# KELVIN-ASU/Lightweight-Multi-Modal-Scene-Understanding-via-Knowledge-Distillation

Hardware: AMD Instinct MI355X
Metric: PandaSet 2-class KD training frames/sec (higher is better)
Workload: dtype f32; 1 GPU; KD step: concat-fusion teacher fwd (eval) -> weighted-fusion student fwd/bwd (train BN), CE + T^2*KL(T=4) + feature-MSE, fused AdamW; random-init weights; teacher_fusion=concat, student_fusion=weighted, image=3x256x256, points_per_frame=80000, bev_grid=64x64, num_classes=2, per_gpu_batch=256, global_batch=256, parallelism=dp1

## Files before the change

### lightweight-multi-modal-scene-understanding-via-knowledge-distillation_amd/csrc/kd_lidar.hip

```cpp
#include "kd_common.h"

namespace {

struct BevGeom { float x0, xd, y0, yd; int H, W; };

__device__ __forceinline__ bool bev_cell(const float4 pt, const BevGeom g, int& cell) {
  const float xn = __fdiv_rn(__fsub_rn(pt.x, g.x0), g.xd);
  const float yn = __fdiv_rn(__fsub_rn(pt.y, g.y0), g.yd);
  const bool valid = (xn >= 0.f) && (xn <= 1.f) && (yn >= 0.f) && (yn <= 1.f);
  if (!valid) { cell = -1; return false; }
  long long ix = (long long)__fmul_rn(xn, (float)(g.W - 1));
  long long iy = (long long)__fmul_rn(yn, (float)(g.H - 1));
  ix = ix < 0 ? 0 : (ix > g.W - 1 ? g.W - 1 : ix);
  iy = iy < 0 ? 0 : (iy > g.H - 1 ? g.H - 1 : iy);
  cell = (int)(iy * g.W + ix);
  return true;
}

struct L0Args {
  const float* pts; const float* w; const float* b; float* y; float* partial;
  int64_t P; int C; int groups, slots; const int* p_dev;
};
__global__ __launch_bounds__(256) void lidar_l0_fwd_kernel(L0Args a) {
  __shared__ float red[2 * 256 * 4];
// ... 364 lines not shown
  const int64_t p = (int64_t)blockIdx.x * blockDim.x + threadIdx.x;
  if (p >= P) return;
  int c;
  if (bev_cell(kd_ld4(pts + p * 4), g, c)) {
    const int row = (int)(p / N) * (g.H * g.W) + c;
    row_of_point[p] = row;
    rank[p] = atomicAdd(counts + row, 1);
  } else {
    row_of_point[p] = -1;
  }
}

__global__ __launch_bounds__(256) void scan_block_sums_kernel(const int* __restrict__ v, int* __restrict__ bsum, int64_t n) {
  __shared__ int red[256];
  const int64_t base = (int64_t)blockIdx.x * SCAN_CHUNK;
  int s = 0;
  for (int i = threadIdx.x; i < SCAN_CHUNK; i += 256)
    if (base + i < n) s += v[base + i];
  red[threadIdx.x] = s;
  __syncthreads();
  for (int off = 128; off > 0; off >>= 1) {
    if ((int)threadIdx.x < off) red[threadIdx.x] += red[threadIdx.x + off];
    __syncthreads();
  }
  if (threadIdx.x == 0) bsum[blockIdx.x] = red[0];
}

__global__ __launch_bounds__(1024) void scan_bsums_kernel(int* bsum, int nb) {
  __shared__ int sh[1024];
  int carry = 0;
  for (int base = 0; base < nb; base += 1024) {
    const int i = base + (int)threadIdx.x;
    const int v = i < nb ? bsum[i] : 0;
    sh[threadIdx.x] = v;
    __syncthreads();
    for (int off = 1; off < 1024; off <<= 1) {
      const int t = (int)threadIdx.x >= off ? sh[threadIdx.x - off] : 0;
      __syncthreads();
      sh[threadIdx.x] += t;
      __syncthreads();
    }
    if (i < nb) bsum[i] = carry + sh[threadIdx.x] - v;
    carry += sh[1023];
    __syncthreads();
  }
}

__global__ __launch_bounds__(256) void scan_apply_kernel(int* v, const int* __restrict__ bsum, int64_t n) {
  __shared__ int sh[256];
  const int64_t base = (int64_t)blockIdx.x * SCAN_CHUNK + (int64_t)threadIdx.x * 8;
  int x[8];
  int tot = 0;
#pragma unroll
  for (int j = 0; j < 8; ++j) { x[j] = base + j < n ? v[base + j] : 0; tot += x[j]; }
  sh[threadIdx.x] = tot;
  __syncthreads();
  for (int off = 1; off < 256; off <<= 1) {
    const int t = (int)threadIdx.x >= off ? sh[threadIdx.x - off] : 0;
    __syncthreads();
    sh[threadIdx.x] += t;
    __syncthreads();
  }
  int run = bsum[blockIdx.x] + sh[threadIdx.x] - tot;
#pragma unroll
  for (int j = 0; j < 8; ++j) {
    if (base + j < n) v[base + j] = run;
    run += x[j];
  }
}

__global__ void seg_fill_kernel(const int* __restrict__ row_of_point, const int* __restrict__ rank,
                                const int* __restrict__ start, int* __restrict__ perm, int64_t P) {
  const int64_t p = (int64_t)blockIdx.x * blockDim.x + threadIdx.x;
  if (p >= P) return;
  const int row = row_of_point[p];
  if (row >= 0) perm[start[row] + rank[p]] = (int)p;
}

constexpr int SORT_BLK = 1024;
constexpr int SORT_MAX_BINS = 36865;

__global__ __launch_bounds__(SORT_BLK) void stable_count_kernel(const float* __restrict__ pts, int* __restrict__ key_out,
                                                                int* __restrict__ lrank_out, int* __restrict__ T, int64_t N,
                                                                int nblk, BevGeom g) {
  extern __shared__ int hist[];
  const int HW = g.H * g.W, nb = HW + 1;
  const int tid = threadIdx.x, lane = tid & 63, wave = tid >> 6;
  const int b = blockIdx.x / nblk, blk = blockIdx.x % nblk;
  for (int i = tid; i < nb; i += SORT_BLK) hist[i] = 0;
  const int64_t n = (int64_t)blk * SORT_BLK + tid;
  const bool act = n < N;
  const int64_t p = (int64_t)b * N + (act ? n : 0);
  int key = -1;
  if (act) {
    int c;
    key = bev_cell(kd_ld4(pts + p * 4), g, c) ? c : HW;
  }
  int r = 0, cnt = 0;
#pragma unroll 16
  for (int j = 0; j < 64; ++j) {
    const int kj = __shfl(key, j);
    cnt += kj == key ? 1 : 0;
    r += (kj == key && j < lane) ? 1 : 0;
  }
  __syncthreads();
  int lr = 0;
  for (int w = 0; w < SORT_BLK / 64; ++w) {
    if (wave == w && act) lr = hist[key] + r;
    __syncthreads();
    if (wave == w && act && r == cnt - 1) hist[key] += cnt;
    __syncthreads();
  }
  if (act) { key_out[p] = key; lrank_out[p] = lr; }
  int* Tb = T + ((int64_t)b * nblk + blk) * nb;
  for (int i = tid; i < nb; i += SORT_BLK) Tb[i] = hist[i];
}

__global__ void stable_prefix_kernel(int* T, int* __restrict__ counts, int* __restrict__ inv, int B, int nblk, int HW) {
  const int nb = HW + 1;
  const int64_t idx = (int64_t)blockIdx.x * blockDim.x + threadIdx.x;
  if (idx == 0) counts[(int64_t)B * HW] = 0;
  if (idx >= (int64_t)B * nb) return;
  const int b = (int)(idx / nb), key = (int)(idx % nb);
  int run = 0;
  for (int blk = 0; blk < nblk; ++blk) {
    int* t = T + ((int64_t)b * nblk + blk) * nb + key;
    const int v = *t;
    *t = run;
    run += v;
  }
  if (key < HW) counts[(int64_t)b * HW + key] = run; else inv[b] = run;
}

__global__ void stable_inv_base_kernel(const int* __restrict__ seg_start, int* inv, int B, int64_t ncells) {
  if (threadIdx.x != 0 || blockIdx.x != 0) return;
  int run = seg_start[ncells];
  for (int b = 0; b < B; ++b) { const int v = inv[b]; inv[b] = run; run += v; }
}

__global__ void stable_fill_kernel(const float* __restrict__ pts, const int* __restrict__ key, const int* __restrict__ lrank,
                                   const int* __restrict__ T, const int* __restrict__ seg_start, const int* __restrict__ inv_base,
                                   float* __restrict__ pts_sorted, int* __restrict__ row_sorted, int* __restrict__ perm,
                                   int64_t P, int64_t N, int nblk, int HW) {
  const int64_t p = (int64_t)blockIdx.x * blockDim.x + threadIdx.x;
  if (p >= P) return;
  const int b = (int)(p / N), blk = (int)((p % N) / SORT_BLK), k = key[p];
  const int base = k < HW ? seg_start[(int64_t)b * HW + k] : inv_base[b];
  const int64_t pos = (int64_t)base + T[((int64_t)b * nblk + blk) * (HW + 1) + k] + lrank[p];
  kd_st4(pts_sorted + pos * 4, kd_ld4(pts + p * 4));
  row_sorted[pos] = k < HW ? b * HW + k : -1;
  if (perm) perm[pos] = (int)p;
}

constexpr int WIDE_MAX_DIM = 4096;

__device__ __forceinline__ void wave_same_key(int key, int lane, int& below, int& all) {
  below = 0; all = 0;
#pragma unroll 16
  for (int j = 0; j < 64; ++j) {
    const int kj = __shfl(key, j);
    all += kj == key ? 1 : 0;
    below += (kj == key && j < lane) ? 1 : 0;
  }
}

__device__ __forceinline__ int block_stable_rank(int key, bool act, int below, int all, int* hist) {
  const int wave = threadIdx.x >> 6;
  int lr = 0;
  for (int w = 0; w < SORT_BLK / 64; ++w) {
    if (wave == w && act) lr = hist[key] + below;
    __syncthreads();
    if (wave == w && act && below == all - 1) hist[key] += all;
    __syncthreads();
  }
  return lr;
}

template <int PASS>
__global__ __launch_bounds__(SORT_BLK) void wide_count_kernel(const float* __restrict__ pts, int* __restrict__ cell_io,
                                                              int* __restrict__ lrank_out, int* __restrict__ T,
                                                              int* counts, int64_t N, int nblk, BevGeom g) {
  extern __shared__ int hist[];
  const int nd = PASS == 0 ? g.W : g.H + 1;
  const int tid = threadIdx.x, lane = tid & 63;
  const int b = blockIdx.x / nblk, blk = blockIdx.x % nblk;
  for (int i = tid; i < nd; i += SORT_BLK) hist[i] = 0;
  const int64_t n = (int64_t)blk * SORT_BLK + tid;
  const bool act = n < N;
  const int64_t p = (int64_t)b * N + (act ? n : 0);
  int cell = -1;
  if (act) {
    if (PASS == 0) bev_cell(kd_ld4(pts + p * 4), g, cell); else cell = cell_io[p];
  }
  const int key = !act ? -1 : PASS == 0 ? (cell >= 0 ? cell % g.W : 0) : (cell >= 0 ? cell / g.W : g.H);
  int below, all;
  wave_same_key(key, lane, below, all);
  if (PASS == 0) {
    int cbelow, call;
    wave_same_key(cell, lane, cbelow, call);
    if (cell >= 0 && cbelow == 0) atomicAdd(counts + (int64_t)b * g.H * g.W + cell, call);
  }
  __syncthreads();
  const int lr = block_stable_rank(key, act, below, all, hist);
  if (act) {
    if (PASS == 0) cell_io[p] = cell;
    lrank_out[p] = lr;
  }
  int* Tb = T + ((int64_t)b * nblk + blk) * nd;
  for (int i = tid; i < nd; i += SORT_BLK) Tb[i] = hist[i];
}

__global__ void wide_prefix_kernel(int* T, int* __restrict__ tot, int* __restrict__ last_tot, int B, int nblk, int nd) {
  const int64_t idx = (int64_t)blockIdx.x * blockDim.x + threadIdx.x;
  if (idx >= (int64_t)B * nd) return;
  const int b = (int)(idx / nd), d = (int)(idx % nd);
  int run = 0;
  for (int blk = 0; blk < nblk; ++blk) {
    int* t = T + ((int64_t)b * nblk + blk) * nd + d;
    const int v = *t;
    *t = run;
    run += v;
  }
  tot[idx] = run;
  if (last_tot && d == nd - 1) last_tot[b] = run;
}

__global__ __launch_bounds__(64) void wide_frame_scan_kernel(int* tot, int nd) {
  int* t = tot + (int64_t)blockIdx.x * nd;
  const int lane = threadIdx.x;
  int carry = 0;
  for (int base = 0; base < nd; base += 64) {
    const int i = base + lane;
    const int v = i < nd ? t[i] : 0;
    int incl = v;
#pragma unroll
    for (int off = 1; off < 64; off <<= 1) {
      const int u = __shfl_up(incl, off);
      if (lane >= off) incl += u;
    }
    if (i < nd) t[i] = carry + incl - v;
    carry += __shfl(incl, 63);
  }
}

__global__ void wide_mid_kernel(const int* __restrict__ cell, const int* __restrict__ lrank, const int* __restrict__ T,
                                const int* __restrict__ off, int* __restrict__ mid_id, int* __restrict__ mid_cell, int64_t P,
                                int64_t N, int nblk, int W) {
  const int64_t p = (int64_t)blockIdx.x * blockDim.x + threadIdx.x;
  if (p >= P) return;
  const int b = (int)(p / N), blk = (int)((p % N) / SORT_BLK), c = cell[p];
  const int d = c >= 0 ? c % W : 0;
  const int64_t pos = (int64_t)b * N + off[(int64_t)b * W + d] + T[((int64_t)b * nblk + blk) * W + d] + lrank[p];
  mid_id[pos] = (int)p;
  mid_cell[pos] = c;
}

__global__ void wide_fill_kernel(const float* __restrict__ pts, const int* __restrict__ mid_id, const int* __restrict__ mid_cell,
                                 const int* __restrict__ lrank, const int* __restrict__ T, const int* __restrict__ off,
                                 const int* __restrict__ seg_start, const int* __restrict__ inv_base,
                                 float* __restrict__ pts_sorted, int* __restrict__ row_sorted, int* __restrict__ perm,
                                 int64_t P, int64_t N, int nblk, int H, int W) {
  const int64_t q = (int64_t)blockIdx.x * blockDim.x + threadIdx.x;
  if (q >= P) return;
  const int b = (int)(q / N), blk = (int)((q % N) / SORT_BLK), c = mid_cell[q], p = mid_id[q];
  const int nd = H + 1, d = c >= 0 ? c / W : H;
  const int64_t HW = (int64_t)H * W;
  const int in_digit = T[((int64_t)b * nblk + blk) * nd + d] + lrank[q];
  const int64_t pos = c >= 0 ? (int64_t)seg_start[b * HW] + off[(int64_t)b * nd + d] + in_digit : (int64_t)inv_base[b] + in_digit;
  kd_st4(pts_sorted + pos * 4, kd_ld4(pts + (int64_t)p * 4));
  row_sorted[pos] = c >= 0 ? (int)(b * HW + c) : -1;
  if (perm) perm[pos] = p;
}

struct SegArgs {
  const float* y; const float* sc; const float* sh; int act;
  const int* start; const int* perm;
  float* grid; const float* dout; const float* mean; const float* invstd;
  float* G; float* partial; int64_t ncells; int C;
  int long_len; const int* rowid; float* cnt; int prow0;
  float* rawmax; uint8_t* holders;
};
constexpr int SEG_LONG = 256;
constexpr int SEG_HOLD_SWEEP = 255;

template <int VEC> struct SegVec;
template <> struct SegVec<1> { typedef float type; };
template <> struct SegVec<2> { typedef float2 type; };
template <> struct SegVec<4> { typedef float4 type; };

template <int VEC> __device__ __forceinline__ void seg_ld(float (&r)[VEC], const float* p) {
  const typename SegVec<VEC>::type v = *reinterpret_cast<const typename SegVec<VEC>::type*>(p);
  __builtin_memcpy(r, &v, sizeof(v));
}
template <int VEC> __device__ __forceinline__ void seg_st(float* p, const float (&r)[VEC]) {
  typename SegVec<VEC>::type v;
  __builtin_memcpy(&v, r, sizeof(v));
  *reinterpret_cast<typename SegVec<VEC>::type*>(p) = v;
}

template <int VEC, bool PERM>
__global__ __launch_bounds__(256) void seg_max_fwd_kernel(SegArgs a) {
  const int lane = threadIdx.x & 63;
  const int c0 = lane * VEC;
  float sc[VEC], sh[VEC];
  seg_ld<VEC>(sc, a.sc + c0);
  seg_ld<VEC>(sh, a.sh + c0);
// ... 287 lines not shown
  seg_stat_rows_out<VEC>(a, red, blockIdx.x, wave, c0, s1, s2);
}

template <int VEC, int MODE>
__global__ __launch_bounds__(256) void seg_long_kernel(SegArgs a) {
  __shared__ float red[4][2][64 * VEC];
  const int lane = threadIdx.x & 63, wave = threadIdx.x >> 6;
  const int c0 = lane * VEC;
  float sc[VEC], sh[VEC], mu[VEC], inv[VEC], s1[VEC], s2[VEC];
  seg_ld<VEC>(sc, a.sc + c0);
  seg_ld<VEC>(sh, a.sh + c0);
#pragma unroll
  for (int j = 0; j < VEC; ++j) { s1[j] = 0.f; s2[j] = 0.f; mu[j] = 0.f; inv[j] = 0.f; }
  if (MODE == 2) { seg_ld<VEC>(mu, a.mean + c0); seg_ld<VEC>(inv, a.invstd + c0); }
  const int nvalid = __builtin_amdgcn_readfirstlane(a.start[a.ncells]);
  const int64_t nw = (int64_t)gridDim.x * 4;
  for (int64_t w = (int64_t)blockIdx.x * 4 + wave; w * 64 < nvalid; w += nw) {
    const int i0 = (int)(w * 64), i1 = i0 + 64 < nvalid ? i0 + 64 : nvalid;
    const int cf = __builtin_amdgcn_readfirstlane(a.rowid[i0]), cl = __builtin_amdgcn_readfirstlane(a.rowid[i1 - 1]);
    const bool lf = a.start[cf + 1] - a.start[cf] > a.long_len, ll = a.start[cl + 1] - a.start[cl] > a.long_len;
    if (!lf && !ll) continue;
    int i = i0;
    while (i < i1) {
      const int cell = __builtin_amdgcn_readfirstlane(a.rowid[i]);
      const int cs = __builtin_amdgcn_readfirstlane(a.start[cell]), ce = __builtin_amdgcn_readfirstlane(a.start[cell + 1]);
      const int rend = ce < i1 ? ce : i1;
      if (ce - cs <= a.long_len) { i = rend; continue; }
      float acc[VEC], mx[VEC], share[VEC];
#pragma unroll
      for (int j = 0; j < VEC; ++j) { acc[j] = 0.f; mx[j] = 0.f; share[j] = 0.f; }
      if (MODE >= 1) seg_ld<VEC>(mx, a.grid + (int64_t)cell * a.C + c0);
      if (MODE == 2) {
        float d[VEC], n[VEC];
        seg_ld<VEC>(d, a.dout + (int64_t)cell * a.C + c0);
        seg_ld<VEC>(n, a.cnt + (int64_t)cell * a.C + c0);
#pragma unroll
        for (int j = 0; j < VEC; ++j) share[j] = n[j] > 0.f ? d[j] / n[j] : 0.f;
        if (i == cs) seg_st<VEC>(a.G + (int64_t)cell * a.C + c0, share);
      }
      int k = i;
      for (; k + 4 <= rend; k += 4) {
        float r[4][VEC];
#pragma unroll
        for (int u = 0; u < 4; ++u) seg_ld<VEC>(r[u], a.y + (int64_t)(k + u) * a.C + c0);
#pragma unroll
        for (int u = 0; u < 4; ++u)
#pragma unroll
          for (int j = 0; j < VEC; ++j) {
            const float v = kd_act(kd_affine(r[u][j], sc[j], sh[j]), a.act);
            if (MODE == 0) acc[j] = v > acc[j] ? v : acc[j];
            if (MODE == 1) acc[j] += (v > 0.f && v == mx[j]) ? 1.f : 0.f;
            if (MODE == 2) {
              const float g = (v > 0.f && v == mx[j]) ? share[j] : 0.f;
              s1[j] += g;
              s2[j] = fmaf(g, (r[u][j] - mu[j]) * inv[j], s2[j]);
            }
          }
      }
      for (; k < rend; ++k) {
        float r[VEC];
        seg_ld<VEC>(r, a.y + (int64_t)k * a.C + c0);
#pragma unroll
        for (int j = 0; j < VEC; ++j) {
          const float v = kd_act(kd_affine(r[j], sc[j], sh[j]), a.act);
          if (MODE == 0) acc[j] = v > acc[j] ? v : acc[j];
          if (MODE == 1) acc[j] += (v > 0.f && v == mx[j]) ? 1.f : 0.f;
          if (MODE == 2) {
            const float g = (v > 0.f && v == mx[j]) ? share[j] : 0.f;
            s1[j] += g;
            s2[j] = fmaf(g, (r[j] - mu[j]) * inv[j], s2[j]);
          }
        }
      }
      if (MODE == 0) {
        unsigned* dst = reinterpret_cast<unsigned*>(a.grid + (int64_t)cell * a.C + c0);
#pragma unroll
        for (int j = 0; j < VEC; ++j)
          if (acc[j] > 0.f) atomicMax(dst + j, __float_as_uint(acc[j]));
      }
      if (MODE == 1) {
#pragma unroll
        for (int j = 0; j < VEC; ++j)
          if (acc[j] > 0.f) atomicAdd(a.cnt + (int64_t)cell * a.C + c0 + j, acc[j]);
      }
      i = rend;
    }
  }
  if (MODE == 2) {
#pragma unroll
    for (int j = 0; j < VEC; ++j) { red[wave][0][c0 + j] = s1[j]; red[wave][1][c0 + j] = s2[j]; }
    __syncthreads();
    for (int i = threadIdx.x; i < 2 * a.C; i += 256) {
      const int st = i / a.C, c = i % a.C;
      a.partial[((int64_t)(a.prow0 + blockIdx.x) * 2 + st) * a.C + c] = red[0][st][c] + red[1][st][c] + red[2][st][c] + red[3][st][c];
    }
  }
}

inline int seg_long_grid(int64_t P) { const int64_t b = (P + 255) / 256; return (int)(b < 1024 ? b : 1024); }

__global__ __launch_bounds__(256) void seg_zero_invalid_kernel(const int* __restrict__ row_of_point, float* __restrict__ G,
                                                               int64_t P, int c4) {
  const int per = 256 / c4;
  const int q = threadIdx.x % c4, sub = threadIdx.x / c4;
  const int64_t base = (int64_t)blockIdx.x * per * 16;
#pragma unroll 4
  for (int k = 0; k < 16; ++k) {
    const int64_t p = base + (int64_t)k * per + sub;
    if (p < P && row_of_point[p] < 0) kd_st4(G + (p * c4 + q) * 4, kd_zero4());
  }
}

__global__ void seg_gather_kernel(const float* __restrict__ pts, const int* __restrict__ perm, const int* __restrict__ row_of_point,
                                  const int* __restrict__ nvalid, float* __restrict__ out_pts, int* __restrict__ out_row, int64_t P) {
  const int64_t i = (int64_t)blockIdx.x * blockDim.x + threadIdx.x;
  if (i >= P || i >= *nvalid) return;
  const int p = perm[i];
  kd_st4(out_pts + i * 4, kd_ld4(pts + (int64_t)p * 4));
  out_row[i] = row_of_point[p];
}

inline int seg_grid(int64_t ncells) { const int64_t b = (ncells + 3) / 4; return (int)(b < 4096 ? b : 4096); }

}

extern "C" {

size_t kd_lidar_cell_sort_ws_bytes(int B, int64_t N, int H, int W) {
  const int64_t n = (int64_t)B * H * W + 1;
  return ((size_t)B * N + (size_t)((n + SCAN_CHUNK - 1) / SCAN_CHUNK)) * sizeof(int);
}

int kd_lidar_cell_sort(const float* pts, int B, int64_t N, int H, int W, float x0, float x1, float y0, float y1,
                       int* row_of_point, int* seg_start, int* perm, void* ws, size_t ws_bytes, void* stream) {
  KD_REQUIRE(pts && row_of_point && seg_start && perm && ws && B > 0 && N > 0 && H > 0 && W > 0, KD_ERR_ARG, "kd_lidar_cell_sort: bad args");
  const int64_t P = (int64_t)B * N, n = (int64_t)B * H * W + 1;
  KD_REQUIRE(P < (int64_t)INT32_MAX && n < (int64_t)INT32_MAX, KD_ERR_SHAPE, "kd_lidar_cell_sort: more than 2^31 points or cells");
  KD_REQUIRE(ws_bytes >= kd_lidar_cell_sort_ws_bytes(B, N, H, W), KD_ERR_WORKSPACE, "kd_lidar_cell_sort: workspace too small");
  hipStream_t st = (hipStream_t)stream;
  int* rank = (int*)ws;
  int* bsum = rank + P;
  const int nb = (int)((n + SCAN_CHUNK - 1) / SCAN_CHUNK);
  hipError_t e = hipMemsetAsync(seg_start, 0, (size_t)n * sizeof(int), st);
  KD_REQUIRE(e == hipSuccess, (int)e, "kd_lidar_cell_sort: memset failed: %s", hipGetErrorString(e));
  const BevGeom g{x0, x1 - x0, y0, y1 - y0, H, W};
  hipLaunchKernelGGL(seg_count_kernel, dim3((unsigned)((P + 255) / 256)), dim3(256), 0, st, pts, row_of_point, rank, seg_start, P, N, g);
  hipLaunchKernelGGL(scan_block_sums_kernel, dim3(nb), dim3(256), 0, st, seg_start, bsum, n);
  hipLaunchKernelGGL(scan_bsums_kernel, dim3(1), dim3(1024), 0, st, bsum, nb);
  hipLaunchKernelGGL(scan_apply_kernel, dim3(nb), dim3(256), 0, st, seg_start, bsum, n);
  hipLaunchKernelGGL(seg_fill_kernel, dim3((unsigned)((P + 255) / 256)), dim3(256), 0, st, row_of_point, rank, seg_start, perm, P);
  return kd_check_launch("kd_lidar_cell_sort");
}

size_t kd_lidar_sort_points_ws_bytes(int B, int64_t N, int H, int W) {
  const int64_t P = (int64_t)B * N, nblk = (N + SORT_BLK - 1) / SORT_BLK, nb = (int64_t)H * W + 1, n = (int64_t)B * H * W + 1;
  return (size_t)(2 * P + (int64_t)B * nblk * nb + B + (n + SCAN_CHUNK - 1) / SCAN_CHUNK) * sizeof(int);
}

int kd_lidar_sort_points(const float* pts, int B, int64_t N, int H, int W, float x0, float x1, float y0, float y1,
                         float* pts_sorted, int* row_sorted, int* seg_start, int* perm, void* ws, size_t ws_bytes,
                         void* stream) {
  KD_REQUIRE(pts && pts_sorted && row_sorted && seg_start && ws && B > 0 && N > 0 && H > 0 && W > 0, KD_ERR_ARG, "kd_lidar_sort_points: bad args");
  const int64_t P = (int64_t)B * N, ncells = (int64_t)B * H * W, n = ncells + 1;
  const int HW = H * W, nb = HW + 1;
  KD_REQUIRE(nb <= SORT_MAX_BINS, KD_ERR_SHAPE, "kd_lidar_sort_points: H*W + 1 = %d bins exceed %d", nb, SORT_MAX_BINS);
  KD_REQUIRE(P < (int64_t)INT32_MAX && n < (int64_t)INT32_MAX, KD_ERR_SHAPE, "kd_lidar_sort_points: more than 2^31 points or cells");
  KD_REQUIRE(ws_bytes >= kd_lidar_sort_points_ws_bytes(B, N, H, W), KD_ERR_WORKSPACE, "kd_lidar_sort_points: workspace too small");
  const int nblk = (int)((N + SORT_BLK - 1) / SORT_BLK);
  KD_REQUIRE((int64_t)B * nblk < (int64_t)INT32_MAX, KD_ERR_SHAPE, "kd_lidar_sort_points: too many blocks");
  hipStream_t st = (hipStream_t)stream;
  int* key = (int*)ws;
  int* lrank = key + P;
  int* T = lrank + P;
  int* inv = T + (int64_t)B * nblk * nb;
  int* bsum = inv + B;
  const int nsb = (int)((n + SCAN_CHUNK - 1) / SCAN_CHUNK);
  const BevGeom g{x0, x1 - x0, y0, y1 - y0, H, W};
  if ((size_t)nb * sizeof(int) > 48 * 1024) {
    hipError_t e = hipFuncSetAttribute(reinterpret_cast<const void*>(stable_count_kernel), hipFuncAttributeMaxDynamicSharedMemorySize,
                                       SORT_MAX_BINS * (int)sizeof(int));
    KD_REQUIRE(e == hipSuccess, (int)e, "kd_lidar_sort_points: cannot raise the LDS limit: %s", hipGetErrorString(e));
  }
  hipLaunchKernelGGL(stable_count_kernel, dim3((unsigned)(B * nblk)), dim3(SORT_BLK), (size_t)nb * sizeof(int), st, pts, key, lrank, T,
                     N, nblk, g);
  const int64_t nbk = (int64_t)B * nb;
  hipLaunchKernelGGL(stable_prefix_kernel, dim3((unsigned)((nbk + 255) / 256)), dim3(256), 0, st, T, seg_start, inv, B, nblk, HW);
  hipLaunchKernelGGL(scan_block_sums_kernel, dim3(nsb), dim3(256), 0, st, seg_start, bsum, n);
  hipLaunchKernelGGL(scan_bsums_kernel, dim3(1), dim3(1024), 0, st, bsum, nsb);
  hipLaunchKernelGGL(scan_apply_kernel, dim3(nsb), dim3(256), 0, st, seg_start, bsum, n);
  hipLaunchKernelGGL(stable_inv_base_kernel, dim3(1), dim3(64), 0, st, seg_start, inv, B, ncells);
  hipLaunchKernelGGL(stable_fill_kernel, dim3((unsigned)((P + 255) / 256)), dim3(256), 0, st, pts, key, lrank, T, seg_start, inv,
                     pts_sorted, row_sorted, perm, P, N, nblk, HW);
  return kd_check_launch("kd_lidar_sort_points");
}

size_t kd_lidar_sort_points_wide_ws_bytes(int B, int64_t N, int H, int W) {
  const int64_t P = (int64_t)B * N, nblk = (N + SORT_BLK - 1) / SORT_BLK, n = (int64_t)B * H * W + 1, nd = (int64_t)W + H + 1;
  return (size_t)(4 * P + (int64_t)B * nblk * nd + (int64_t)B * nd + B + (n + SCAN_CHUNK - 1) / SCAN_CHUNK) * sizeof(int);
}

int kd_lidar_sort_points_wide(const float* pts, int B, int64_t N, int H, int W, float x0, float x1, float y0, float y1,
                              float* pts_sorted, int* row_sorted, int* seg_start, int* perm, void* ws, size_t ws_bytes,
                              void* stream) {
  KD_REQUIRE(pts && pts_sorted && row_sorted && seg_start && ws && B > 0 && N > 0 && H > 0 && W > 0, KD_ERR_ARG, "kd_lidar_sort_points_wide: bad args");
  KD_REQUIRE(H <= WIDE_MAX_DIM && W <= WIDE_MAX_DIM, KD_ERR_SHAPE, "kd_lidar_sort_points_wide: grid %d x %d exceeds %d cells per side", H, W,
             WIDE_MAX_DIM);
  const int64_t P = (int64_t)B * N, ncells = (int64_t)B * H * W, n = ncells + 1;
  KD_REQUIRE(P < (int64_t)INT32_MAX && n < (int64_t)INT32_MAX, KD_ERR_SHAPE, "kd_lidar_sort_points_wide: more than 2^31 points or cells");
  KD_REQUIRE(ws_bytes >= kd_lidar_sort_points_wide_ws_bytes(B, N, H, W), KD_ERR_WORKSPACE, "kd_lidar_sort_points_wide: workspace too small");
  const int nblk = (int)((N + SORT_BLK - 1) / SORT_BLK);
  KD_REQUIRE((int64_t)B * nblk < (int64_t)INT32_MAX, KD_ERR_SHAPE, "kd_lidar_sort_points_wide: too many blocks");
  hipStream_t st = (hipStream_t)stream;
  const int nd0 = W, nd1 = H + 1;
  int* cell = (int*)ws;
  int* lrank = cell + P;
  int* mid_id = lrank + P;
  int* mid_cell = mid_id + P;
  int* T0 = mid_cell + P;
  int* T1 = T0 + (int64_t)B * nblk * nd0;
  int* off0 = T1 + (int64_t)B * nblk * nd1;
  int* off1 = off0 + (int64_t)B * nd0;
  int* inv = off1 + (int64_t)B * nd1;
  int* bsum = inv + B;
  const int nsb = (int)((n + SCAN_CHUNK - 1) / SCAN_CHUNK);
  const BevGeom g{x0, x1 - x0, y0, y1 - y0, H, W};
  hipError_t e = hipMemsetAsync(seg_start, 0, (size_t)n * sizeof(int), st);
  KD_REQUIRE(e == hipSuccess, (int)e, "kd_lidar_sort_points_wide: memset failed: %s", hipGetErrorString(e));
  const dim3 blocks((unsigned)(B * nblk)), per_point((unsigned)((P + 255) / 256));
  hipLaunchKernelGGL(wide_count_kernel<0>, blocks, dim3(SORT_BLK), (size_t)nd0 * sizeof(int), st, pts, cell, lrank, T0, seg_start, N, nblk, g);
  hipLaunchKernelGGL(wide_prefix_kernel, dim3((unsigned)(((int64_t)B * nd0 + 255) / 256)), dim3(256), 0, st, T0, off0, (int*)nullptr, B, nblk, nd0);
  hipLaunchKernelGGL(wide_frame_scan_kernel, dim3(B), dim3(64), 0, st, off0, nd0);
  hipLaunchKernelGGL(wide_mid_kernel, per_point, dim3(256), 0, st, cell, lrank, T0, off0, mid_id, mid_cell, P, N, nblk, W);
  hipLaunchKernelGGL(wide_count_kernel<1>, blocks, dim3(SORT_BLK), (size_t)nd1 * sizeof(int), st, (const float*)nullptr, mid_cell, lrank, T1,
                     (int*)nullptr, N, nblk, g);
  hipLaunchKernelGGL(wide_prefix_kernel, dim3((unsigned)(((int64_t)B * nd1 + 255) / 256)), dim3(256), 0, st, T1, off1, inv, B, nblk, nd1);
  hipLaunchKernelGGL(wide_frame_scan_kernel, dim3(B), dim3(64), 0, st, off1, nd1);
  hipLaunchKernelGGL(scan_block_sums_kernel, dim3(nsb), dim3(256), 0, st, seg_start, bsum, n);
  hipLaunchKernelGGL(scan_bsums_kernel, dim3(1), dim3(1024), 0, st, bsum, nsb);
  hipLaunchKernelGGL(scan_apply_kernel, dim3(nsb), dim3(256), 0, st, seg_start, bsum, n);
  hipLaunchKernelGGL(stable_inv_base_kernel, dim3(1), dim3(64), 0, st, seg_start, inv, B, ncells);
  hipLaunchKernelGGL(wide_fill_kernel, per_point, dim3(256), 0, st, pts, mid_id, mid_cell, lrank, T1, off1, seg_start, inv, pts_sorted,
                     row_sorted, perm, P, N, nblk, H, W);
  return kd_check_launch("kd_lidar_sort_points_wide");
}

int kd_lidar_gather_sorted(const float* pts, const int* perm, const int* row_of_point, const int* nvalid_dev, float* out_pts,
                           int* out_row, int64_t P, void* stream) {
  KD_REQUIRE(pts && perm && row_of_point && nvalid_dev && out_pts && out_row && P > 0, KD_ERR_ARG, "kd_lidar_gather_sorted: bad args");
  hipLaunchKernelGGL(seg_gather_kernel, dim3((unsigned)((P + 255) / 256)), dim3(256), 0, (hipStream_t)stream, pts, perm, row_of_point,
                     nvalid_dev, out_pts, out_row, P);
  return kd_check_launch("kd_lidar_gather_sorted");
}

int kd_lidar_seg_max_fwd(const float* y, const float* sc, const float* sh, int act, const int* seg_start, const int* perm,
                         const int* row_sorted, float* grid, int64_t P, int64_t ncells, int C, void* stream) {
  KD_REQUIRE(y && sc && sh && seg_start && grid && ncells > 0, KD_ERR_ARG, "kd_lidar_seg_max_fwd: bad args");
  KD_REQUIRE(C == 64 || C == 128 || C == 256, KD_ERR_SHAPE, "kd_lidar_seg_max_fwd: C must be 64, 128 or 256 (got %d)", C);
  KD_REQUIRE(act == KD_ACT_RELU || act == KD_ACT_RELU6, KD_ERR_ARG, "kd_lidar_seg_max_fwd: needs a non-negative activation");
  const bool chunked = row_sorted != nullptr && perm == nullptr && P > 0;
  SegArgs a{y, sc, sh, act, seg_start, perm, grid, nullptr, nullptr, nullptr, nullptr, nullptr, ncells, C,
            chunked ? SEG_LONG : 0, row_sorted, nullptr, 0};
  const dim3 gr(seg_grid(ncells)), bl(256);
  hipStream_t st = (hipStream_t)stream;
#define KD_SEG_LAUNCH(kern)                                                                          \
  do {                                                                                              \
    if (C == 64) { if (perm) hipLaunchKernelGGL((kern<1, true>), gr, bl, 0, st, a); else hipLaunchKernelGGL((kern<1, false>), gr, bl, 0, st, a); } \
    else if (C == 128) { if (perm) hipLaunchKernelGGL((kern<2, true>), gr, bl, 0, st, a); else hipLaunchKernelGGL((kern<2, false>), gr, bl, 0, st, a); } \
    else { if (perm) hipLaunchKernelGGL((kern<4, true>), gr, bl, 0, st, a); else hipLaunchKernelGGL((kern<4, false>), gr, bl, 0, st, a); } \
  } while (0)
  KD_SEG_LAUNCH(seg_max_fwd_kernel);
  if (chunked) {
    const dim3 gl(seg_long_grid(P));
    if (C == 64) hipLaunchKernelGGL((seg_long_kernel<1, 0>), gl, bl, 0, st, a);
    else if (C == 128) hipLaunchKernelGGL((seg_long_kernel<2, 0>), gl, bl, 0, st, a);
    else hipLaunchKernelGGL((seg_long_kernel<4, 0>), gl, bl, 0, st, a);
  }
  return kd_check_launch("kd_lidar_seg_max_fwd");
}

int64_t kd_lidar_seg_stat_rows(int64_t ncells) { return seg_grid(ncells); }

int kd_lidar_seg_max_bwd(const float* y, const float* sc, const float* sh, int act, const float* grid, const float* dout,
                         const float* mean, const float* invstd, const int* seg_start, const int* perm,
                         const int* row_of_point, float* G, float* partial, int64_t P, int64_t ncells, int C, void* stream) {
  KD_REQUIRE(y && sc && sh && grid && dout && mean && invstd && seg_start && row_of_point && G && partial && P > 0 && ncells > 0,
             KD_ERR_ARG, "kd_lidar_seg_max_bwd: bad args");
  KD_REQUIRE(act != KD_ACT_RELU6, KD_ERR_ARG, "kd_lidar_seg_max_bwd: ReLU6 is not supported in the scatter-max backward (a saturated maximum has derivative 0; the holder split here is ReLU's)");
  KD_REQUIRE(C == 64 || C == 128 || C == 256, KD_ERR_SHAPE, "kd_lidar_seg_max_bwd: C must be 64, 128 or 256 (got %d)", C);
  SegArgs a{y, sc, sh, act, seg_start, perm, const_cast<float*>(grid), dout, mean, invstd, G, partial, ncells, C, 0, nullptr, nullptr, 0};
  const dim3 gr(seg_grid(ncells)), bl(256);
  hipStream_t st = (hipStream_t)stream;
  const int c4 = C / 4;
  const int64_t per_block = (int64_t)(256 / c4) * 16;
  hipLaunchKernelGGL(seg_zero_invalid_kernel, dim3((unsigned)((P + per_block - 1) / per_block)), dim3(256), 0, st, row_of_point, G, P, c4);
  KD_SEG_LAUNCH(seg_max_bwd_kernel);
#undef KD_SEG_LAUNCH
  return kd_check_launch("kd_lidar_seg_max_bwd");
}

int64_t kd_lidar_seg_share_stat_rows(int64_t ncells, int64_t P) { return seg_grid(ncells) + seg_long_grid(P); }

int kd_lidar_seg_share_bwd(const float* y, const float* sc, const float* sh, int act, const float* grid, const float* dout,
                           const float* mean, const float* invstd, const int* seg_start, const int* row_sorted, float* share,
                           float* cnt_ws, float* partial, int64_t P, int64_t ncells, int C, void* stream) {
  KD_REQUIRE(y && sc && sh && grid && dout && mean && invstd && seg_start && row_sorted && share && cnt_ws && partial && ncells > 0 && P > 0,
             KD_ERR_ARG, "kd_lidar_seg_share_bwd: bad args");
  KD_REQUIRE(act != KD_ACT_RELU6, KD_ERR_ARG, "kd_lidar_seg_share_bwd: ReLU6 is not supported in the scatter-max backward (a saturated maximum has derivative 0; the holder split here is ReLU's)");
  KD_REQUIRE(C == 64 || C == 128 || C == 256, KD_ERR_SHAPE, "kd_lidar_seg_share_bwd: C must be 64, 128 or 256 (got %d)", C);
  SegArgs a{y, sc, sh, act, seg_start, nullptr, const_cast<float*>(grid), dout, mean, invstd, share, partial, ncells, C,
            SEG_LONG, row_sorted, cnt_ws, seg_grid(ncells)};
  const dim3 gr(seg_grid(ncells)), gl(seg_long_grid(P)), bl(256);
  hipStream_t st = (hipStream_t)stream;
  if (C == 64) {
    hipLaunchKernelGGL((seg_max_bwd_kernel<1, false, true>), gr, bl, 0, st, a);
    hipLaunchKernelGGL((seg_long_kernel<1, 1>), gl, bl, 0, st, a);
    hipLaunchKernelGGL((seg_long_kernel<1, 2>), gl, bl, 0, st, a);
  } else if (C == 128) {
    hipLaunchKernelGGL((seg_max_bwd_kernel<2, false, true>), gr, bl, 0, st, a);
    hipLaunchKernelGGL((seg_long_kernel<2, 1>), gl, bl, 0, st, a);
    hipLaunchKernelGGL((seg_long_kernel<2, 2>), gl, bl, 0, st, a);
  } else {
    hipLaunchKernelGGL((seg_max_bwd_kernel<4, false, true>), gr, bl, 0, st, a);
    hipLaunchKernelGGL((seg_long_kernel<4, 1>), gl, bl, 0, st, a);
    hipLaunchKernelGGL((seg_long_kernel<4, 2>), gl, bl, 0, st, a);
  }
  return kd_check_launch("kd_lidar_seg_share_bwd");
}

int kd_lidar_seg_hold_fwd(const float* y, const float* sc, const float* sh, int act, const int* seg_start, const int* row_sorted,
                          float* grid, float* rawmax, uint8_t* holders, int64_t P, int64_t ncells, int C, void* stream) {
  KD_REQUIRE(y && sc && sh && seg_start && row_sorted && grid && rawmax && holders && ncells > 0 && P > 0, KD_ERR_ARG,
             "kd_lidar_seg_hold_fwd: bad args");
  KD_REQUIRE(C == 64 || C == 128 || C == 256, KD_ERR_SHAPE, "kd_lidar_seg_hold_fwd: C must be 64, 128 or 256 (got %d)", C);
  KD_REQUIRE(act == KD_ACT_RELU || act == KD_ACT_RELU6, KD_ERR_ARG, "kd_lidar_seg_hold_fwd: needs a non-negative activation");
  KD_REQUIRE((uintptr_t)holders % 4 == 0, KD_ERR_ARG, "kd_lidar_seg_hold_fwd: holders must be 4-byte aligned");
  SegArgs a{y, sc, sh, act, seg_start, nullptr, grid, nullptr, nullptr, nullptr, nullptr, nullptr, ncells, C,
            SEG_LONG, row_sorted, nullptr, 0, rawmax, holders};
// ... 46 lines not shown
```

Measured before the change: 3574 frames/s.

## Sort lidar points per frame with one block per frame and wave-ballot ranking

Adds a per-frame sort path for large batches: one block per frame builds a histogram of BEV cells in LDS, then a fill kernel computes global offsets in-block and scatters points, using ballot-based key-match masks to rank same-key lanes within a wave. This replaces the seven-kernel pipeline (count, prefix, multi-pass scans, inv base, fill) and its large workspace tables, cutting launches and global traffic. Within-frame order follows wave-serialized atomics, so it stays stable per chunk only if the wave loop is ordered as written. Parallelism is limited to B blocks, and each block serially walks 80k points twice.

```diff
diff --git a/lightweight-multi-modal-scene-understanding-via-knowledge-distillation_amd/csrc/kd_lidar.hip b/lightweight-multi-modal-scene-understanding-via-knowledge-distillation_amd/csrc/kd_lidar.hip
--- a/lightweight-multi-modal-scene-understanding-via-knowledge-distillation_amd/csrc/kd_lidar.hip
+++ b/lightweight-multi-modal-scene-understanding-via-knowledge-distillation_amd/csrc/kd_lidar.hip
@@ -540,6 +540,154 @@
   if (perm) perm[pos] = (int)p;
 }
 
+constexpr int SORT_PPT = 4;
+constexpr int SORT_CHUNK = SORT_BLK * SORT_PPT;
+
+__device__ __forceinline__ void wave_key_masks(const int (&key)[SORT_PPT], int nbits, unsigned long long (&m)[SORT_PPT]) {
+  unsigned dlo[SORT_PPT], dhi[SORT_PPT];
+#pragma unroll
+  for (int s = 0; s < SORT_PPT; ++s) dlo[s] = dhi[s] = 0;
+  for (int b = 0; b < nbits; ++b) {
+#pragma unroll
+    for (int s = 0; s < SORT_PPT; ++s) {
+      const unsigned bit = (unsigned)(key[s] >> b) & 1u;
+      const unsigned long long set = __ballot(bit);
+      const unsigned t = 0u - bit;
+      dlo[s] |= (unsigned)set ^ t;
+      dhi[s] |= (unsigned)(set >> 32) ^ t;
+    }
+  }
+#pragma unroll
+  for (int s = 0; s < SORT_PPT; ++s) m[s] = ~(((unsigned long long)dhi[s] << 32) | dlo[s]);
+}
+
+__device__ __forceinline__ void frame_chunk_keys(const float* __restrict__ fp, int64_t base, int64_t N, const BevGeom g, int wave,
+                                                 int lane, float4 (&pt)[SORT_PPT], int (&key)[SORT_PPT]) {
+#pragma unroll
+  for (int s = 0; s < SORT_PPT; ++s) {
+    const int64_t n = base + (wave * SORT_PPT + s) * 64 + lane;
+    key[s] = g.H * g.W + 1;
+    pt[s] = kd_zero4();
+    if (n < N) {
+      pt[s] = kd_ld4(fp + n * 4);
+      int c;
+      key[s] = bev_cell(pt[s], g, c) ? c : g.H * g.W;
+    }
+  }
+}
+
+__global__ __launch_bounds__(SORT_BLK) void frame_count_kernel(const float* __restrict__ pts, int* __restrict__ counts,
+                                                               int* __restrict__ inv, int64_t N, BevGeom g) {
+  extern __shared__ int hist[];
+  const int HW = g.H * g.W, nb = HW + 1;
+  const int tid = threadIdx.x, lane = tid & 63, wave = __builtin_amdgcn_readfirstlane(tid >> 6);
+  const int b = blockIdx.x;
+  for (int i = tid; i < nb; i += SORT_BLK) hist[i] = 0;
+  __syncthreads();
+  const float* fp = pts + (int64_t)b * N * 4;
+  for (int64_t base = 0; base < N; base += SORT_CHUNK) {
+    float4 pt[SORT_PPT];
+    int key[SORT_PPT];
+    frame_chunk_keys(fp, base, N, g, wave, lane, pt, key);
+#pragma unroll
+    for (int s = 0; s < SORT_PPT; ++s)
+      if (key[s] <= HW) atomicAdd(&hist[key[s]], 1);
+  }
+  __syncthreads();
+  int* cb = counts + (int64_t)b * HW;
+  for (int i = tid; i < HW; i += SORT_BLK) cb[i] = hist[i];
+  if (tid == 0) inv[b] = hist[HW];
+}
+
+__global__ __launch_bounds__(SORT_BLK) void frame_fill_kernel(const float* __restrict__ pts, int* __restrict__ seg_start,
+                                                              const int* __restrict__ inv, float* __restrict__ pts_sorted,
+                                                              int* __restrict__ row_sorted, int* __restrict__ perm, int64_t N,
+                                                              BevGeom g) {
+  extern __shared__ int run[];
+  __shared__ int wsum[SORT_BLK / 64], inv_sum[2];
+  const int HW = g.H * g.W, nbits = 32 - __clz(HW + 1);
+  const int tid = threadIdx.x, lane = tid & 63, wave = __builtin_amdgcn_readfirstlane(tid >> 6);
+  const int b = blockIdx.x, B = gridDim.x;
+  int* start = seg_start + (int64_t)b * HW;
+  for (int i = tid; i < HW; i += SORT_BLK) run[i] = start[i];
+  if (tid < 2) inv_sum[tid] = 0;
+  __syncthreads();
+  int below = 0, all = 0;
+  for (int f = tid; f < B; f += SORT_BLK) { const int v = inv[f]; all += v; below += f < b ? v : 0; }
+  if (below) atomicAdd(&inv_sum[0], below);
+  if (all) atomicAdd(&inv_sum[1], all);
+  const int per = (HW + SORT_BLK - 1) / SORT_BLK;
+  const int i0 = min(tid * per, HW), i1 = min(i0 + per, HW);
+  int mine = 0;
+  for (int i = i0; i < i1; ++i) mine += run[i];
+  int incl = mine;
+#pragma unroll
+  for (int off = 1; off < 64; off <<= 1) {
+    const int t = __shfl_up(incl, off);
+    if (lane >= off) incl += t;
+  }
+  if (lane == 63) wsum[wave] = incl;
+  __syncthreads();
+  const int n_valid = (int)((int64_t)B * N - inv_sum[1]);
+  int pos0 = (int)((int64_t)b * N - inv_sum[0]) + incl - mine;
+  for (int w = 0; w < wave; ++w) pos0 += wsum[w];
+  for (int i = i0; i < i1; ++i) { const int c = run[i]; run[i] = pos0; pos0 += c; }
+  if (tid == 0) {
+    run[HW] = n_valid + inv_sum[0];
+    if (b == 0) seg_start[(int64_t)B * HW] = n_valid;
+  }
+  __syncthreads();
+  for (int i = tid; i < HW; i += SORT_BLK) start[i] = run[i];
+  const int frame_end = (int)((int64_t)b * N - inv_sum[0]) + (int)N - inv[b];
+  for (int k0 = wave * 64; k0 < HW; k0 += SORT_BLK) {
+    const int k = k0 + lane;
+    const int end = k + 1 < HW ? run[k + 1] : frame_end;
+    const int q1 = __builtin_amdgcn_readlane(end, 63);
+    for (int q0 = __builtin_amdgcn_readfirstlane(run[k0]); q0 < q1; q0 += 64) {
+      const int q = q0 + lane;
+      int j = 0;
+#pragma unroll
+      for (int step = 32; step > 0; step >>= 1)
+        if (__shfl(end, j + step - 1) <= q) j += step;
+      if (q < q1) row_sorted[q] = b * HW + k0 + j;
+    }
+  }
+  for (int q = run[HW] + tid, q1 = run[HW] + inv[b]; q < q1; q += SORT_BLK) row_sorted[q] = -1;
+  __syncthreads();
+
+  const float* fp = pts + (int64_t)b * N * 4;
+  for (int64_t base = 0; base < N; base += SORT_CHUNK) {
+    float4 pt[SORT_PPT];
+    int key[SORT_PPT], rank[SORT_PPT], lead[SORT_PPT], cnt[SORT_PPT], pos[SORT_PPT];
+    unsigned long long m[SORT_PPT];
+    frame_chunk_keys(fp, base, N, g, wave, lane, pt, key);
+    wave_key_masks(key, nbits, m);
+#pragma unroll
+    for (int s = 0; s < SORT_PPT; ++s) {
+      rank[s] = __popcll(m[s] & ((1ull << lane) - 1ull));
+      lead[s] = __ffsll(m[s]) - 1;
+      cnt[s] = __popcll(m[s]);
+      pos[s] = 0;
+    }
+    for (int w = 0; w < SORT_BLK / 64; ++w) {
+      if (wave == w) {
+#pragma unroll
+        for (int s = 0; s < SORT_PPT; ++s)
+          if (key[s] <= HW && lane == lead[s]) pos[s] = atomicAdd(&run[key[s]], cnt[s]);
+      }
+      __syncthreads();
+    }
+#pragma unroll
+    for (int s = 0; s < SORT_PPT; ++s) {
+      const int64_t q = (int64_t)__shfl(pos[s], lead[s]) + rank[s];
+      if (key[s] <= HW) {
+        kd_st4(pts_sorted + q * 4, pt[s]);
+        if (perm) perm[q] = (int)((int64_t)b * N + base + (wave * SORT_PPT + s) * 64 + lane);
+      }
+    }
+  }
+}
+
 constexpr int WIDE_MAX_DIM = 4096;
 
 __device__ __forceinline__ void wave_same_key(int key, int lane, int& below, int& all) {
@@ -1133,7 +1281,15 @@
   return kd_check_launch("kd_lidar_cell_sort");
 }
 
+constexpr int SORT_FRAME_MIN_B = 64;
+constexpr int SORT_FRAME_SMALL_N = SORT_CHUNK, SORT_FRAME_SMALL_HW = 4096;
+static bool sort_by_frame(int B, int64_t N, int H, int W) {
+  const int64_t HW = (int64_t)H * W;
+  return HW + 1 <= SORT_MAX_BINS && (B >= SORT_FRAME_MIN_B || (N <= SORT_FRAME_SMALL_N && HW <= SORT_FRAME_SMALL_HW));
+}
+
 size_t kd_lidar_sort_points_ws_bytes(int B, int64_t N, int H, int W) {
+  if (sort_by_frame(B, N, H, W)) return (size_t)B * sizeof(int);
   const int64_t P = (int64_t)B * N, nblk = (N + SORT_BLK - 1) / SORT_BLK, nb = (int64_t)H * W + 1, n = (int64_t)B * H * W + 1;
   return (size_t)(2 * P + (int64_t)B * nblk * nb + B + (n + SCAN_CHUNK - 1) / SCAN_CHUNK) * sizeof(int);
 }
@@ -1147,23 +1303,36 @@
   KD_REQUIRE(nb <= SORT_MAX_BINS, KD_ERR_SHAPE, "kd_lidar_sort_points: H*W + 1 = %d bins exceed %d", nb, SORT_MAX_BINS);
   KD_REQUIRE(P < (int64_t)INT32_MAX && n < (int64_t)INT32_MAX, KD_ERR_SHAPE, "kd_lidar_sort_points: more than 2^31 points or cells");
   KD_REQUIRE(ws_bytes >= kd_lidar_sort_points_ws_bytes(B, N, H, W), KD_ERR_WORKSPACE, "kd_lidar_sort_points: workspace too small");
+  hipStream_t st = (hipStream_t)stream;
+  const BevGeom g{x0, x1 - x0, y0, y1 - y0, H, W};
+  const size_t lds = (size_t)nb * sizeof(int);
+  if (sort_by_frame(B, N, H, W)) {
+    int* inv = (int*)ws;
+    if (lds > 48 * 1024) {
+      static std::atomic<uint64_t> count_raised{0}, fill_raised{0};
+      hipError_t e = kd_raise_dynamic_lds(reinterpret_cast<const void*>(frame_count_kernel), SORT_MAX_BINS * sizeof(int), count_raised);
+      if (e == hipSuccess)
+        e = kd_raise_dynamic_lds(reinterpret_cast<const void*>(frame_fill_kernel), SORT_MAX_BINS * sizeof(int), fill_raised);
+      KD_REQUIRE(e == hipSuccess, (int)e, "kd_lidar_sort_points: cannot raise the LDS limit: %s", hipGetErrorString(e));
+    }
+    hipLaunchKernelGGL(frame_count_kernel, dim3((unsigned)B), dim3(SORT_BLK), lds, st, pts, seg_start, inv, N, g);
+    hipLaunchKernelGGL(frame_fill_kernel, dim3((unsigned)B), dim3(SORT_BLK), lds, st, pts, seg_start, inv, pts_sorted, row_sorted, perm, N, g);
+    return kd_check_launch("kd_lidar_sort_points");
+  }
   const int nblk = (int)((N + SORT_BLK - 1) / SORT_BLK);
   KD_REQUIRE((int64_t)B * nblk < (int64_t)INT32_MAX, KD_ERR_SHAPE, "kd_lidar_sort_points: too many blocks");
-  hipStream_t st = (hipStream_t)stream;
   int* key = (int*)ws;
   int* lrank = key + P;
   int* T = lrank + P;
   int* inv = T + (int64_t)B * nblk * nb;
   int* bsum = inv + B;
   const int nsb = (int)((n + SCAN_CHUNK - 1) / SCAN_CHUNK);
-  const BevGeom g{x0, x1 - x0, y0, y1 - y0, H, W};
-  if ((size_t)nb * sizeof(int) > 48 * 1024) {
-    hipError_t e = hipFuncSetAttribute(reinterpret_cast<const void*>(stable_count_kernel), hipFuncAttributeMaxDynamicSharedMemorySize,
-                                       SORT_MAX_BINS * (int)sizeof(int));
+  if (lds > 48 * 1024) {
+    static std::atomic<uint64_t> raised{0};
+    const hipError_t e = kd_raise_dynamic_lds(reinterpret_cast<const void*>(stable_count_kernel), SORT_MAX_BINS * sizeof(int), raised);
     KD_REQUIRE(e == hipSuccess, (int)e, "kd_lidar_sort_points: cannot raise the LDS limit: %s", hipGetErrorString(e));
   }
-  hipLaunchKernelGGL(stable_count_kernel, dim3((unsigned)(B * nblk)), dim3(SORT_BLK), (size_t)nb * sizeof(int), st, pts, key, lrank, T,
-                     N, nblk, g);
+  hipLaunchKernelGGL(stable_count_kernel, dim3((unsigned)(B * nblk)), dim3(SORT_BLK), lds, st, pts, key, lrank, T, N, nblk, g);
   const int64_t nbk = (int64_t)B * nb;
   hipLaunchKernelGGL(stable_prefix_kernel, dim3((unsigned)((nbk + 255) / 256)), dim3(256), 0, st, T, seg_start, inv, B, nblk, HW);
   hipLaunchKernelGGL(scan_block_sums_kernel, dim3(nsb), dim3(256), 0, st, seg_start, bsum, n);
```

Measured after the change: 3606 frames/s, median of 6. No clear change (+0.9%).
